# hku-mars/ImMesh

Measured on AMD Instinct MI355X. Metric: scans/sec (reg+mesh), 100k-pt scan into 10M-voxel map, higher is better.
Workload: dtype f64

## Files before the change

immesh_amd/csrc/c_api.cpp:

```cpp
#include "host_ctx.hpp"
#include "imu_host.hpp"
#include <cmath>
#include <new>

#define RP_ABORTED 1
static thread_local std::string g_create_error;
thread_local KProf* g_kprof = nullptr;



extern "C" {

void immesh_default_config(immesh_config* c) {
    std::memset(c, 0, sizeof(*c));
    c->voxel_size = 0.5; c->max_layer = 2;
    for (int i = 0; i < 5; i++) c->layer_init[i] = 5;
    c->max_points_size = 100; c->planer_threshold = 0.01; c->dept_err = 0.02; c->beam_err = 0.05; c->calib_laser = 0;
    c->sigma_num = 3.0; c->max_iter = 4;
    c->extR[0] = c->extR[4] = c->extR[8] = 1.0;
    c->extT[0] = 0.04165; c->extT[1] = 0.02326; c->extT[2] = -0.0284;
    c->mesh_min_spacing = 0.1; c->mesh_voxel = 0.4; c->mesh_region = 10.0; c->mesh_append_budget = 10000;
}

const char* immesh_create_error(void) { return g_create_error.c_str(); }
// ... 36 lines not shown

    const int64_t ns = g.cap_scan_points > 0 ? g.cap_scan_points : 600000;
    c->cap_scan = ns;
    A(c->d_pts_down, ns * 3); A(c->d_pts_raw, ns * 4);
    A(c->d_partials, ((ns + 63) / 64) * RES_NR); A(c->d_out48, RES_NV); A(c->d_done, 4);
    HIPCHK(c, hipMemsetAsync(c->d_done, 0, 16, c->stream));
    A(c->d_match, ns); A(c->d_mnode, ns); A(c->d_dis, ns); A(c->d_rinv, ns); A(c->d_normal, ns * 3);
    A(c->d_ptdata, ns * IM_PT_DOUBLES);
    A(c->d_key_a, ns); A(c->d_key_b, ns); A(c->d_idx_a, ns); A(c->d_idx_b, ns); A(c->d_idx_c, ns);
    A(c->d_slot, ns); A(c->d_slot_s, ns); A(c->d_seg_start, ns); A(c->d_nseg, 16); A(c->d_ds_out, ns * 3);
    c->sort_temp_bytes = std::max({sort_pairs_u64_temp_bytes((int)ns), sort_pairs_u32_temp_bytes((int)ns), exclusive_sum_temp_bytes((int)ns)}) + 256;
    { char* t; A(t, c->sort_temp_bytes); c->d_sort_temp = t; }
    A(c->p_key_a, ns); A(c->p_key_b, ns); A(c->p_idx_a, ns); A(c->p_idx_b, ns); A(c->p_idx_c, ns); A(c->p_seg, ns); A(c->p_nseg, 16); A(c->p_slot, ns); A(c->p_slot_s, ns); A(c->p_pool4, ns * 4);
    { char* t; A(t, c->sort_temp_bytes); c->p_sort_temp = t; }
    {
        unsigned long long cap = 1024; while (cap < 2ull * (unsigned long long)ns) cap <<= 1;
        char* t; A(t, cap * 16); c->p_htab = t; c->p_htab_cap = cap;
        launch_ds_table_reset(c->stream, t, cap);
        if ((rc = c->pinned(&c->h_ds_dyn, &c->d_ds_dyn, 1)) || (rc = c->pinned(&c->h_ds_info, &c->d_ds_info, 16))) return rc;
        HIPCHK(c, hipMemsetAsync(c->p_nseg, 0, 16 * sizeof(int32_t), c->stream));
    }
    {
        m.split_general = c->knobs.split_general >= 0 ? c->knobs.split_general : (g.max_layer >= 3 ? 1 : 0);
        A(m.sub_order, ns); A(m.sub_items, 2 * ns);
        HIPCHK(c, hipMemsetAsync(m.sub_items, 0, (size_t)2 * ns * sizeof(unsigned long long), c->stream));
    }
    A(c->d_dump_count, 2);
    A(c->d_touched, 2 * ns + 16);
    A(c->d_regstate, 1);
    A(c->d_epi, 8);
    HIPCHK(c, hipMemsetAsync(c->d_epi, 0, 32, c->stream));
    for (int q = 0; q < 2; q++) { A(c->d_rp_slots[q], RP_SLOT_DOUBLES); launch_fill_u64(c->stream, (unsigned long long*)c->d_rp_slots[q], RP_SLOT_SENTINEL, RP_SLOT_DOUBLES); }
    HIPCHK(c, hipMemsetAsync(c->d_regstate, 0, sizeof(RegState), c->stream));
    A(c->d_und_in, ns * 5); A(c->d_und_out, ns * 4); A(c->d_und_tab, 64 * 23 + 24);
#undef A
    if ((rc = c->pinned(&c->h_out48, &c->d_out48_host, RES_NV)) || (rc = c->pinned(&c->h_reg_out, &c->d_reg_out_host, REG_OUT_DOUBLES)) ||
        (rc = c->pinned(&c->h_epi_flag, &c->d_epi_flag_host, 8)) || (rc = c->pinned(&c->h_counters, &c->d_counters_host, 16))) return rc;
    return 0;
}


immesh_ctx* immesh_create(const immesh_config* cfg) {
    g_create_error.clear();
    if (!cfg) { g_create_error = "null config"; return nullptr; }
    int ndev = 0;
    hipError_t e = hipGetDeviceCount(&ndev);
// ... 678 lines not shown
```

immesh_amd/csrc/host_knobs.hpp:

```cpp
#pragma once
#include <hip/hip_runtime.h>
#include <algorithm>
#include <cstdlib>
#include <cstring>
#include <string>

struct Knobs {
    bool debug = false;
    bool debug_waits = false;
    std::string trace_file;
    int split_general = -1;
    bool no_priority = false;
    int mesh_cus = 0;
    int rp_blocks = 0;
    bool rp_force_abort = false;
    bool match_seq = false;
    bool host_ekf = false;
    bool serial_safe = false;
    bool serial_order = false;
    bool ds_radix = false;
    bool ds_no_gate = false;
    bool no_graph = false;
    int split_mode = 2;
    int mesh_room = 0;
    bool no_pipeline = false;
    int tri_stream = 1;
    int fused_wgs = 768;
    int list_div = 0;
    int mesh_grid_div = 1;

    static Knobs from_env(int mesh_npar) {
        auto on = [](const char* name) { return getenv(name) != nullptr; };
        auto num = [](const char* name, int unset) { const char* e = getenv(name); return e ? atoi(e) : unset; };
        Knobs k;
        k.debug = on("IMMESH_DEBUG"); k.debug_waits = on("IMMESH_DEBUG_WAITS");
        if (const char* e = getenv("IMMESH_TRACE_FILE")) k.trace_file = e;
        if (on("IMMESH_SPLIT_GENERAL")) k.split_general = num("IMMESH_SPLIT_GENERAL", 0);
        k.no_priority = on("IMMESH_NO_PRIORITY");
        k.mesh_cus = num("IMMESH_MESH_CUS", 0); if (k.mesh_cus < 8 || k.mesh_cus >= 1024) k.mesh_cus = 0;
        if (on("IMMESH_RP_BLOCKS")) k.rp_blocks = std::max(1, num("IMMESH_RP_BLOCKS", 0));
        k.rp_force_abort = on("IMMESH_RP_FORCE_ABORT"); k.match_seq = on("IMMESH_MATCH_SEQ"); k.host_ekf = on("IMMESH_HOST_EKF");
        k.serial_safe = on("IMMESH_SERIAL_SAFE"); k.serial_order = on("IMMESH_SERIAL_ORDER");
        k.ds_radix = on("IMMESH_DS_RADIX"); k.ds_no_gate = on("IMMESH_DS_NO_GATE");
        k.no_graph = on("IMMESH_NO_GRAPH");
        k.split_mode = on("IMMESH_NO_SPLIT") ? 0 : 2;
        if (on("IMMESH_SPLIT")) k.split_mode = num("IMMESH_SPLIT", 0) == 0 ? 0 : 1;
        if (on("IMMESH_MESH_ROOM")) k.mesh_room = std::min(std::max(num("IMMESH_MESH_ROOM", 0), 1), mesh_npar);
        k.no_pipeline = on("IMMESH_NO_PIPELINE");
        k.tri_stream = num("IMMESH_TRI_STREAM", 1);
        { const int v = num("IMMESH_FUSED_WGS", 0); k.fused_wgs = v >= 32 ? v : 768; }
        { const int v = num("IMMESH_LIST_DIV", 0); k.list_div = v >= 4 ? v : 0; }
        k.mesh_grid_div = std::max(1, num("IMMESH_MESH_GRID_DIV", 1));
        return k;
    }

    hipError_t make_stream(hipStream_t* s, int priority, bool maskable) const {
        if (!maskable || !mesh_cus) return hipStreamCreateWithPriority(s, hipStreamNonBlocking, priority);
        uint32_t mask[32];
        std::memset(mask, 0, sizeof(mask));
        for (int i = 0; i < mesh_cus; i++) mask[i >> 5] |= 1u << (i & 31);
        return hipExtStreamCreateWithCUMask(s, 32, mask);
    }
};
```

immesh_amd/csrc/reg_kernels.hip:

```cpp
#include <algorithm>
#include <cstdlib>
#include "regmap.hpp"
#include "kernels.hpp"
#include "prof.hpp"

using namespace imd;

struct PlaneRegs { double n[3], c[3], pv[21]; float d, radius; };
struct BestMatch { int node; int layer; double prob; bool ok; PlaneRegs P; };

IMD double plane_sigma(const double* pv, const double* J) {
    double tmp[6];
#pragma unroll
    for (int c = 0; c < 6; c++) {
        double s = 0;
#pragma unroll
        for (int r = 0; r < 6; r++) s += J[r] * pv[(r <= c) ? sym21_index(r, c) : sym21_index(c, r)];
        tmp[c] = s;
    }
    double sig = 0;
#pragma unroll
    for (int c = 0; c < 6; c++) sig += tmp[c] * J[c];
    return sig;
}
// ... 1184 lines not shown
#pragma unroll
        for (int k = 0; k < 3; k++) t[k] = q->t[k];
        transform_point(sp.extR, sp.extT, R, t, raw, world, i);
        return;
    }
    const int i = blockIdx.x * blockDim.x + threadIdx.x;
    if (i >= n) return;
    if (spd) {
#pragma unroll
        for (int k = 0; k < 9; k++) { sp.R[k] = spd->R[k]; sp.RextR[k] = spd->RextR[k]; sp.rot_var[k] = spd->rot_var[k]; sp.t_var[k] = spd->t_var[k]; }
#pragma unroll
        for (int k = 0; k < 3; k++) sp.t[k] = spd->t[k];
    }
    point_var_point(m, sp, pts, i, stride, mode, pt_data, sort_key, slot_out, pt_next);
}

__global__ void segment_heads_kernel(const uint32_t* __restrict__ sorted_slot, int n, int32_t* __restrict__ seg_start, int32_t* __restrict__ nseg) {
    const int i = blockIdx.x * blockDim.x + threadIdx.x;
    if (i >= n) return;
    if (sorted_slot[i] == 0xFFFFFFFFu) return;
    if (i == 0 || sorted_slot[i - 1] != sorted_slot[i]) seg_start[atomicAdd(nseg, 1)] = i;
}

struct WaveCtx { int lane; int64_t* stats; int root; bool shared = false; };

struct PlaneFit { double c[3], ev[3], U[9]; int imin, imax; bool planar; };
IMD double sel3(const int i, const double a, const double b, const double c) { return i == 0 ? a : (i == 1 ? b : c); }

template <class FE>
IMD void fit_eigen(FE&& for_each_point, const int n, const float planer_threshold, PlaneFit& f) {
    double s[9];
#pragma unroll
    for (int k = 0; k < 9; k++) s[k] = 0;
    for_each_point([&](const double* q) __attribute__((always_inline)) {
        const double x = q[0], y = q[1], z = q[2];
        s[0] += x; s[1] += y; s[2] += z;
        s[3] += x * x; s[4] += x * y; s[5] += x * z; s[6] += y * y; s[7] += y * z; s[8] += z * z;
    });
#pragma unroll
    for (int k = 0; k < 9; k++) s[k] = wave_sum_fast(s[k]);
    const double dn = (double)n;
    f.c[0] = s[0] / dn; f.c[1] = s[1] / dn; f.c[2] = s[2] / dn;
    double cov[9];
    cov[0] = s[3] / dn - f.c[0] * f.c[0]; cov[1] = s[4] / dn - f.c[0] * f.c[1]; cov[2] = s[5] / dn - f.c[0] * f.c[2];
    cov[3] = cov[1];                      cov[4] = s[6] / dn - f.c[1] * f.c[1]; cov[5] = s[7] / dn - f.c[1] * f.c[2];
    cov[6] = cov[2];                      cov[7] = cov[5];                      cov[8] = s[8] / dn - f.c[2] * f.c[2];
// ... 75 lines not shown
        const double Umin[3] = {sel3(imin, f.U[0], f.U[1], f.U[2]), sel3(imin, f.U[3], f.U[4], f.U[5]), sel3(imin, f.U[6], f.U[7], f.U[8])};
        if (lane < 21) {
            double v = 0;
#pragma unroll
            for (int k = 0; k < 21; k++) if (lane == k) v = pv[k];
            nr.p_var[lane] = v;
        }
        if (lane == 0) {
            const double evmin = sel3(imin, f.ev[0], f.ev[1], f.ev[2]);
            const double evmax = sel3(f.imax, f.ev[0], f.ev[1], f.ev[2]);
#pragma unroll
            for (int k = 0; k < 3; k++) { nr.p_center[k] = f.c[k]; nr.p_normal[k] = Umin[k]; }
            nr.min_eig = (float)evmin;
            nr.radius = (float)sqrt(evmax);
            nr.d = (float)(-(Umin[0] * f.c[0] + Umin[1] * f.c[1] + Umin[2] * f.c[2]));
        }
    } else if (lane == 0) {
#pragma unroll
        for (int k = 0; k < 3; k++) { nr.p_center[k] = f.c[k]; nr.p_normal[k] = 0.0; }
        nr.radius = 0.f;
    }
}

__device__ __noinline__ bool wave_init_plane(const RegMapDev& m, int nd, int n, const WaveCtx& w) {
    __builtin_amdgcn_fence(__ATOMIC_ACQUIRE, "workgroup");
    if (w.lane == 0 && w.stats) { atomicAdd((unsigned long long*)&w.stats[0], 1ull); atomicAdd((unsigned long long*)&w.stats[1], (unsigned long long)n); }
    PlaneFit f;
    double pv[21];
    const int lane = w.lane;
    if (n <= 128) {
        double P0[9], P1[9];
#pragma unroll
        for (int k = 0; k < 9; k++) { P0[k] = 0; P1[k] = 0; }
        if (lane < n) { const double* q = node_point_ptr(m, nd, lane);
#pragma unroll
            for (int k = 0; k < 9; k++) P0[k] = q[k]; }
        if (lane + 64 < n) { const double* q = node_point_ptr(m, nd, lane + 64);
#pragma unroll
            for (int k = 0; k < 9; k++) P1[k] = q[k]; }
        auto fe = [&](auto&& fn) __attribute__((always_inline)) { if (lane < n) fn(P0); if (lane + 64 < n) fn(P1); };
        fit_eigen(fe, n, m.planer_threshold, f);
        if (f.planar) fit_plane_var(fe, n, f, pv);
    } else {
        auto fe = [&](auto&& fn) __attribute__((always_inline)) {
            for (int i = lane; i < n; i += 64) {
                const double* q = node_point_ptr(m, nd, i);
                double P[9];
#pragma unroll
                for (int k = 0; k < 9; k++) P[k] = q[k];
                fn(P);
            }
        };
        fit_eigen(fe, n, m.planer_threshold, f);
        if (f.planar) fit_plane_var(fe, n, f, pv);
    }
    fit_store(m.nodes[nd], f, pv, lane);
    return f.planar;
}

__device__ bool wave_push_point(const RegMapDev& m, int nd, int n, const double* src, const WaveCtx& w) {
    int ok = 1;
    if (w.lane == 0 && (n % IM_CHUNK_PTS) == 0) ok = node_ensure_chunk(m, nd, n / IM_CHUNK_PTS) ? 1 : 0;
    ok = __shfl(ok, 0, 64);
    if (!ok) return false;
    __builtin_amdgcn_fence(__ATOMIC_RELEASE, "workgroup");
    __builtin_amdgcn_fence(__ATOMIC_ACQUIRE, "workgroup");
    if (w.lane < IM_PT_DOUBLES) {
        double* dst = node_point_ptr(m, nd, n);
        dst[w.lane] = src[w.lane];
    }
    __builtin_amdgcn_fence(__ATOMIC_RELEASE, "workgroup");
    return true;
}

IMD int octant_of(const double* q, const double* center) {
    return 4 * (q[0] > center[0] ? 1 : 0) + 2 * (q[1] > center[1] ? 1 : 0) + (q[2] > center[2] ? 1 : 0);
}
IMD int make_child(const RegMapDev& m, int nd, int oct) {
    const float ql = m.nodes[nd].quarter;
    const int xyz[3] = {(oct >> 2) & 1, (oct >> 1) & 1, oct & 1};
    double c[3];
#pragma unroll
    for (int k = 0; k < 3; k++) c[k] = m.nodes[nd].center[k] + (double)((float)(2 * xyz[k] - 1) * ql);
    const int layer = m.nodes[nd].layer + 1;
    const int child = node_alloc(m, layer, c, ql / 2, m.nodes[nd].key, m.nodes[nd].path | (oct << (3 * (layer - 1))));
    m.nodes[nd].child[oct] = child;
    return child;
}

__device__ void wave_init_octo_tree(const RegMapDev& m, int node, int* stack, const WaveCtx& w) {
    int sp = 0;
    if (w.lane == 0) stack[0] = node;
    sp = 1;
    while (sp > 0) {
        __builtin_amdgcn_fence(__ATOMIC_ACQUIRE, "workgroup");
        const int nd = __shfl(stack[sp - 1], 0, 64);
        sp--;
        const int n = m.nodes[nd].npts;
        const bool planar = wave_init_plane(m, nd, n, w);
        const int layer = m.nodes[nd].layer;
        if (w.lane == 0) {
            const int f0 = m.nodes[nd].flags;
            int f = f0 | NF_INIT;
            f = planar ? (f | NF_PLANE) : (f & ~NF_PLANE);
            node_set_flags(m, w.root, nd, f0, f, w.shared);
            m.nodes[nd].newpts = 0;
        }
        if (planar || layer >= m.max_layer) continue;
        const double ctr[3] = {m.nodes[nd].center[0], m.nodes[nd].center[1], m.nodes[nd].center[2]};
        int child_id[8], child_n[8];
#pragma unroll
        for (int k = 0; k < 8; k++) { child_id[k] = m.nodes[nd].child[k]; child_n[k] = child_id[k] >= 0 ? m.nodes[child_id[k]].npts : 0; }
        for (int base = 0; base < n; base += 64) {
// ... 24 lines not shown
#pragma unroll
                    for (int e = 0; e < IM_PT_DOUBLES; e++) dst[e] = q[e];
                }
                child_n[k] += cnt;
            }
        }
        __builtin_amdgcn_fence(__ATOMIC_RELEASE, "workgroup");
        if (w.lane == 0) {
#pragma unroll
            for (int k = 0; k < 8; k++)
                if (child_id[k] >= 0) { m.nodes[child_id[k]].npts = child_n[k]; m.nodes[child_id[k]].newpts = child_n[k]; }
            node_free_points(m, nd);
        }
#pragma unroll
        for (int k = 7; k >= 0; k--)
            if (child_id[k] >= 0 && child_n[k] > m.init_size[min(layer + 1, 4)]) {
                if (w.lane == 0) stack[sp] = child_id[k];
                sp++;
            }
        __builtin_amdgcn_fence(__ATOMIC_RELEASE, "workgroup");
    }
}

__device__ void wave_update_point(const RegMapDev& m, int root, const double* src, int* stack, const WaveCtx& w) {
    int nd = root;
    for (int depth = 0; depth < 8; depth++) {
        __builtin_amdgcn_fence(__ATOMIC_ACQUIRE, "workgroup");
        const int flags = m.nodes[nd].flags;
        const int layer = m.nodes[nd].layer;
        const int n = m.nodes[nd].npts;
        if (!(flags & NF_INIT)) {
            if (!wave_push_point(m, nd, n, src, w)) return;
            if (w.lane == 0) { m.nodes[nd].npts = n + 1; m.nodes[nd].newpts = m.nodes[nd].newpts + 1; }
            __builtin_amdgcn_fence(__ATOMIC_RELEASE, "workgroup");
            if (n + 1 > m.init_size[min(layer, 4)]) wave_init_octo_tree(m, nd, stack, w);
            return;
        }
        if (flags & NF_PLANE) {
            if (!(flags & NF_UPDATE_EN)) return;
            if (!wave_push_point(m, nd, n, src, w)) return;
            int newp = m.nodes[nd].newpts + 1;
            if (w.lane == 0) m.nodes[nd].npts = n + 1;
            __builtin_amdgcn_fence(__ATOMIC_RELEASE, "workgroup");
            if (newp > 5) {
                const bool planar = wave_init_plane(m, nd, n + 1, w);
                if (w.lane == 0) node_set_flags(m, w.root, nd, flags, planar ? (flags | NF_PLANE) : (flags & ~NF_PLANE), w.shared);
                newp = 0;
// ... 23 lines not shown
            if (child < 0) return;
            nd = child;
            continue;
        }
        if (!(flags & NF_UPDATE_EN)) return;
        if (!wave_push_point(m, nd, n, src, w)) return;
        int newp = m.nodes[nd].newpts + 1;
        if (w.lane == 0) m.nodes[nd].npts = n + 1;
        __builtin_amdgcn_fence(__ATOMIC_RELEASE, "workgroup");
        if (newp > 5) {
            const bool planar = wave_init_plane(m, nd, n + 1, w);
            if (w.lane == 0) node_set_flags(m, w.root, nd, flags, planar ? (flags | NF_PLANE) : (flags & ~NF_PLANE), w.shared);
            newp = 0;
        }
        if (w.lane == 0) {
            m.nodes[nd].newpts = newp;
            if (n + 1 > IM_G_MAX_POINTS) { m.nodes[nd].flags = m.nodes[nd].flags & ~NF_UPDATE_EN; node_free_points(m, nd); }
        }
        __builtin_amdgcn_fence(__ATOMIC_RELEASE, "workgroup");
        return;
    }
}

__device__ int wave_replay_planar_root(const RegMapDev& m, const int root, const int* order, const int cnt, const double* __restrict__ pt_data, const WaveCtx& w) {
    NodeRec& nd = m.nodes[root];
    int flags = nd.flags;
    const int layer = nd.layer;
    int npts = nd.npts, newp = nd.newpts;
    const int want = NF_INIT | NF_PLANE | NF_UPDATE_EN;
    if (layer == 0 && (flags & want) == (NF_INIT | NF_PLANE)) return cnt;
    if ((flags & want) != want || layer != 0 || npts + cnt > IM_INLINE_CHUNKS * IM_CHUNK_PTS) return 0;
    int chunks[IM_INLINE_CHUNKS];
#pragma unroll
    for (int k = 0; k < IM_INLINE_CHUNKS; k++) chunks[k] = nd.chunks[k];
    auto chunk_of = [&](int ci) { int c = chunks[0];
#pragma unroll
        for (int k = 1; k < IM_INLINE_CHUNKS; k++) { const int ck = chunks[k]; c = (ci == k) ? ck : c; }
        return c; };
    double s1[3] = {0, 0, 0}, s2[3] = {0, 0, 0};
    const bool will_refit = newp + cnt > 5;
    if (will_refit) {
        for (int i = w.lane; i < npts; i += 64) {
            const double* q = m.chunk_data + ((size_t)chunk_of(i / IM_CHUNK_PTS) * IM_CHUNK_PTS + (i % IM_CHUNK_PTS)) * IM_PT_DOUBLES;
#pragma unroll
            for (int a = 0; a < 3; a++) { const double v = q[a]; s1[a] += v; s2[a] += v * v; }
        }
#pragma unroll
// ... 57 lines not shown
                    }
                    j++;
                    break;
                }
            }
        }
        if (npts >= m.max_points_size) {
            if (last_refit_n) { write_header(); (void)wave_init_plane(m, root, last_refit_n, wq); last_refit_n = 0; }
            flags &= ~NF_UPDATE_EN;
            write_header();
            if (w.lane == 0) { node_free_points(m, root); nd.newpts = 0; }
            __builtin_amdgcn_fence(__ATOMIC_RELEASE, "workgroup");
            npts = 0; newp = 0;
            j++;
            break;
        }
    }
    if (header_dirty) write_header();
    if (last_refit_n) (void)wave_init_plane(m, root, last_refit_n, wq);
    if (w.lane == 0 && w.stats && n_ref) { atomicAdd((unsigned long long*)&w.stats[0], (unsigned long long)n_ref); atomicAdd((unsigned long long*)&w.stats[1], (unsigned long long)n_ref_pts); }
    return j;
}

__device__ int wave_replay_planar_node(const RegMapDev& m, const int node, const int* order, const int cnt, const double* __restrict__ pt_data, const WaveCtx& w) {
    NodeRec& nd = m.nodes[node];
    int flags = nd.flags;
    const int want = NF_INIT | NF_PLANE | NF_UPDATE_EN;
    if ((flags & want) == (NF_INIT | NF_PLANE)) return cnt;
    if ((flags & want) != want) return 0;
    int npts = nd.npts, newp = nd.newpts;
    double s1[3] = {0, 0, 0}, s2[3] = {0, 0, 0};
    const bool will_refit = newp + cnt > 5;
    if (will_refit) {
        for (int i = w.lane; i < npts; i += 64) {
            const double* q = node_point_ptr(m, node, i);
#pragma unroll
            for (int a = 0; a < 3; a++) { const double v = q[a]; s1[a] += v; s2[a] += v * v; }
        }
#pragma unroll
        for (int a = 0; a < 3; a++) { s1[a] = wave_sum(s1[a]); s2[a] = wave_sum(s2[a]); }
    }
    WaveCtx wq = w; wq.stats = nullptr;
    int last_refit_n = 0, n_ref = 0, j = 0;
    long long n_ref_pts = 0;
    auto write_counts = [&]() {
        if (w.lane == 0) { nd.npts = npts; nd.newpts = newp; }
        __builtin_amdgcn_fence(__ATOMIC_RELEASE, "workgroup");
// ... 67 lines not shown
    if (root < 0) return;
    w.root = root;
    if (mode == 0) {
        for (int j = start; j < n && sorted_slot[j] == slot; j++)
            wave_update_point(m, root, pt_data + (size_t)sorted_idx[j] * IM_PT_DOUBLES, stacks[wv], w);
    } else {
        int cnt = m.nodes[root].npts;
        for (int j = start; j < n && sorted_slot[j] == slot; j++) {
            if (!wave_push_point(m, root, cnt, pt_data + (size_t)sorted_idx[j] * IM_PT_DOUBLES, w)) return;
            cnt++;
        }
        if (w.lane == 0) { m.nodes[root].npts = cnt; m.nodes[root].newpts = cnt; }
        __builtin_amdgcn_fence(__ATOMIC_RELEASE, "workgroup");
        if (cnt > m.init_size[0]) wave_init_octo_tree(m, root, stacks[wv], w);
    }
}

#define RL_CAP 64
#define DBG_FUSED_OFF 64
#define DBG_FUSED_RECS 16384
#define DBG_RES_OFF (DBG_FUSED_OFF + DBG_FUSED_RECS * 8)
static_assert(DBG_RES_OFF + 8 * 512 * 8 == REG_DBG_WORDS, "the IMMESH_DEBUG buffer (kernels.hpp) holds the counters and both trace areas");
#define RF_PTS 128
__global__ __launch_bounds__(256, 3) void replay_fused_kernel(RegMapDev m, const int32_t* __restrict__ pt_next, const unsigned long long* __restrict__ sort_key,
                                                            const double* __restrict__ pt_data, int64_t* stats, uint32_t* __restrict__ general_list,
                                                            unsigned long long* __restrict__ dbg, unsigned long long* flag_dev, unsigned long long* flag_host,
                                                            unsigned long long flag_seq) {
    if (flag_dev && blockIdx.x == 0 && threadIdx.x == 0) {
        __hip_atomic_store(flag_dev, flag_seq, __ATOMIC_RELAXED, __HIP_MEMORY_SCOPE_AGENT);
        __hip_atomic_store(flag_host, flag_seq, __ATOMIC_RELAXED, __HIP_MEMORY_SCOPE_SYSTEM);
    }
    __shared__ unsigned long long skey[4][RL_CAP];
    __shared__ int sidx[4][RL_CAP];
    __shared__ int order[4][RL_CAP];
    __builtin_amdgcn_s_setprio(REG_UPD_PRIO);
    const int wv = threadIdx.x >> 6, lane = threadIdx.x & 63;
    const int t_first = blockIdx.x * 4 + wv, t_stride = gridDim.x * 4;
    uint32_t slot_first = m.touched[2 * (size_t)t_first];
    int root_first = (int)m.touched[2 * (size_t)t_first + 1];
    const int n_touched = m.counters[7];
#define FDBG(k) do { if (dbg) { const unsigned long long _t = __builtin_readcyclecounter(); if (tr) ((unsigned int*)tr)[4 + (k)] = (unsigned int)(_t - tprev); tprev = _t; } } while (0)
#define FEND(state, nref) do { if (tr) { tr[1] = __builtin_amdgcn_s_memrealtime(); tr[7] = (unsigned long long)((unsigned)cnt | ((unsigned)(nref) << 8) | ((unsigned)(state) << 16)); } } while (0)
    auto process = [&](const int t, const uint32_t slot, int root) __attribute__((always_inline)) {
    unsigned long long* const tr = (dbg && lane == 0 && t < DBG_FUSED_RECS) ? dbg + DBG_FUSED_OFF + (size_t)t * 8 : nullptr;
    unsigned long long tprev = dbg ? __builtin_readcyclecounter() : 0;
    if (tr) { tr[0] = __builtin_amdgcn_s_memrealtime(); tr[2] = tr[3] = tr[4] = tr[5] = tr[6] = tr[7] = 0; }
    if (root < 0) root = m.htab[slot].root;
    if (root < 0) return;
    FDBG(0);
    NodeRec& nd = m.nodes[root];
    const int flags = nd.flags, layer = nd.layer;
    const int npts = nd.npts, newp = nd.newpts;
    if (dbg) { asm volatile("s_waitcnt vmcnt(0)" ::: "memory"); FDBG(1); }
    int chunks[IM_INLINE_CHUNKS];
#pragma unroll
    for (int k = 0; k < IM_INLINE_CHUNKS; k++) chunks[k] = nd.chunks[k];
    if (dbg) { asm volatile("s_waitcnt vmcnt(0)" ::: "memory"); FDBG(2); }
    int cnt = 0;
    int ihead = (int)(unsigned int)(m.slot_head[slot] & 0xFFFFFFFFull);
    if (dbg) { asm volatile("s_waitcnt vmcnt(0)" ::: "memory"); FDBG(3); }
    for (int i = ihead; i >= 0; i = pt_next[i]) {
        if (cnt < RL_CAP && lane == 0) { skey[wv][cnt] = sort_key[i]; sidx[wv][cnt] = i; }
        cnt++;
    }
    FDBG(4);
    const int want = NF_INIT | NF_PLANE | NF_UPDATE_EN;
    if (layer == 0 && (flags & want) == (NF_INIT | NF_PLANE)) { FEND(1, 0); return; }
    const int ntot = npts + cnt;
    bool hand_over = cnt > RL_CAP || (flags & want) != want || layer != 0 || newp > 5 || ntot > RF_PTS || ntot >= m.max_points_size;
    if (!hand_over) {
        __builtin_amdgcn_fence(__ATOMIC_RELEASE, "workgroup");
        __builtin_amdgcn_wave_barrier();
        __builtin_amdgcn_fence(__ATOMIC_ACQUIRE, "workgroup");
        for (int e = lane; e < cnt; e += 64) {
            const unsigned long long k = skey[wv][e];
            const int id = sidx[wv][e];
            int rank = 0;
            for (int f = 0; f < cnt; f++) { const unsigned long long kf = skey[wv][f]; rank += (kf < k || (kf == k && sidx[wv][f] < id)) ? 1 : 0; }
            order[wv][rank] = id;
        }
        __builtin_amdgcn_fence(__ATOMIC_RELEASE, "workgroup");
        __builtin_amdgcn_wave_barrier();
        __builtin_amdgcn_fence(__ATOMIC_ACQUIRE, "workgroup");
        FDBG(5);
        auto chunk_of = [&](int ci) { int c = chunks[0];
#pragma unroll
            for (int k = 1; k < IM_INLINE_CHUNKS; k++) { const int ck = chunks[k]; c = (ci == k) ? ck : c; }
            return c; };
        const int n_ref = (newp + cnt) / 6;
        double P0[9], P1[9];
#pragma unroll
        for (int k = 0; k < 9; k++) { P0[k] = 0; P1[k] = 0; }
        {
// ... 54 lines not shown
                    for (int k = 0; k < 9; k++) d[k] = P0[k]; }
                if (q1 >= npts && q1 < ntot) { double* d = m.chunk_data + ((size_t)chunk_of(q1 >> 4) * IM_CHUNK_PTS + (q1 & 15)) * IM_PT_DOUBLES;
#pragma unroll
                    for (int k = 0; k < 9; k++) d[k] = P1[k]; }
            }
            if (lane == 0) {
                nd.npts = ntot; nd.newpts = (newp + cnt) % 6;
#pragma unroll
                for (int k = 0; k < IM_INLINE_CHUNKS; k++) nd.chunks[k] = chunks[k];
                if (n_ref) { int64_t* sh = stats + 16 + (size_t)(t & 63) * 16; atomicAdd((unsigned long long*)&sh[0], (unsigned long long)n_ref); atomicAdd((unsigned long long*)&sh[1], (unsigned long long)n_ref_pts); }
            }
            FDBG(8);
            if (n_ref > 0) {
                double pv[21];
                auto fe = [&](auto&& fn) __attribute__((always_inline)) { if (lane < n_last) fn(P0); if (lane + 64 < n_last) fn(P1); };
                fit_plane_var(fe, n_last, fit, pv);
                fit_store(nd, fit, pv, lane);
            }
            FDBG(9);
            FEND(2, n_ref);
            return;
        }
    }
    if (lane == 0) general_list[atomicAdd(&m.counters[10], 1)] = slot;
    FEND(3, 0);
    };
    for (int t = t_first; t < n_touched; t += t_stride) {
        if (t != t_first) { slot_first = m.touched[2 * (size_t)t]; root_first = (int)m.touched[2 * (size_t)t + 1]; }
        process(t, slot_first, root_first);
    }
#undef FDBG
#undef FEND
}

__device__ bool replay_split_root(const RegMapDev& m, const int root, const int* order, const int cnt, const double* __restrict__ pt_data, const WaveCtx& w);
__device__ bool replay_split_leaves(const RegMapDev& m, const int root, const int* order, const int cnt, const double* __restrict__ pt_data, const WaveCtx& w, int* s_key, int* s_first);
__global__ __launch_bounds__(256) void replay_list_kernel(RegMapDev m, const int32_t* __restrict__ pt_next, const unsigned long long* __restrict__ sort_key,
                                                           const double* __restrict__ pt_data, int64_t* stats, int32_t* __restrict__ big_idx, int32_t* __restrict__ big_order,
                                                           unsigned long long* __restrict__ dbg, const uint32_t* __restrict__ work, const int32_t* __restrict__ n_work) {
    __shared__ unsigned long long skey[4][RL_CAP];
    __shared__ int sidx[4][RL_CAP];
    __shared__ int order[4][RL_CAP];
    __shared__ int stacks[4][48];
    __builtin_amdgcn_s_setprio(REG_UPD_PRIO);
    const int wv = threadIdx.x >> 6;
    const int nw = *n_work;
    WaveCtx w; w.lane = threadIdx.x & 63; w.stats = stats;
    for (int t = blockIdx.x * 4 + wv; t < nw; t += gridDim.x * 4) {
        const uint32_t slot = work[t];
        const int root = m.htab[slot].root;
        if (root < 0) continue;
        w.root = root;
        const unsigned long long tdbg0 = dbg ? __builtin_readcyclecounter() : 0;
        __builtin_amdgcn_wave_barrier();
        int cnt = 0;
        for (int i = (int)(unsigned int)(m.slot_head[slot] & 0xFFFFFFFFull); i >= 0; i = pt_next[i]) {
            if (cnt < RL_CAP && w.lane == 0) { skey[wv][cnt] = sort_key[i]; sidx[wv][cnt] = i; }
            cnt++;
        }
        if (cnt > RL_CAP) {
            int base = 0;
            if (w.lane == 0) base = atomicAdd(&m.counters[9], cnt);
            base = __shfl(base, 0, 64);
            if (w.lane == 0) { int k = 0; for (int i = (int)(unsigned int)(m.slot_head[slot] & 0xFFFFFFFFull); i >= 0; i = pt_next[i]) big_idx[base + k++] = i; }
            __builtin_amdgcn_fence(__ATOMIC_RELEASE, "agent");
            __builtin_amdgcn_wave_barrier();
            __builtin_amdgcn_fence(__ATOMIC_ACQUIRE, "agent");
            for (int e = w.lane; e < cnt; e += 64) {
                const int id = big_idx[base + e];
                const unsigned long long k = sort_key[id];
                int rank = 0;
                for (int f = 0; f < cnt; f++) { const int idf = big_idx[base + f]; const unsigned long long kf = sort_key[idf]; rank += (kf < k || (kf == k && idf < id)) ? 1 : 0; }
                big_order[base + rank] = id;
            }
            __builtin_amdgcn_fence(__ATOMIC_RELEASE, "agent");
            __builtin_amdgcn_wave_barrier();
            __builtin_amdgcn_fence(__ATOMIC_ACQUIRE, "agent");
            if (replay_split_root(m, root, big_order + base, cnt, pt_data, w)) continue;
            int jb = wave_replay_planar_root(m, root, big_order + base, cnt, pt_data, w);
            if (jb == 0) jb = wave_replay_planar_node(m, root, big_order + base, cnt, pt_data, w);
            for (int j = jb; j < cnt; j++) wave_update_point(m, root, pt_data + (size_t)big_order[base + j] * IM_PT_DOUBLES, stacks[wv], w);
            continue;
        }
        __builtin_amdgcn_fence(__ATOMIC_RELEASE, "workgroup");
        __builtin_amdgcn_wave_barrier();
        __builtin_amdgcn_fence(__ATOMIC_ACQUIRE, "workgroup");
        for (int e = w.lane; e < cnt; e += 64) {
            const unsigned long long k = skey[wv][e];
            const int id = sidx[wv][e];
            int rank = 0;
            for (int f = 0; f < cnt; f++) { const unsigned long long kf = skey[wv][f]; rank += (kf < k || (kf == k && sidx[wv][f] < id)) ? 1 : 0; }
            order[wv][rank] = id;
        }
        __builtin_amdgcn_fence(__ATOMIC_RELEASE, "workgroup");
        __builtin_amdgcn_wave_barrier();
        __builtin_amdgcn_fence(__ATOMIC_ACQUIRE, "workgroup");
        if (replay_split_leaves(m, root, order[wv], cnt, pt_data, w, (int*)skey[wv], sidx[wv])) continue;
        if (replay_split_root(m, root, order[wv], cnt, pt_data, w)) continue;
        const unsigned long long tdbg1 = dbg ? __builtin_readcyclecounter() : 0;
        int jf = wave_replay_planar_root(m, root, order[wv], cnt, pt_data, w);
        if (jf == 0) jf = wave_replay_planar_node(m, root, order[wv], cnt, pt_data, w);
        for (int j = jf; j < cnt; j++) wave_update_point(m, root, pt_data + (size_t)order[wv][j] * IM_PT_DOUBLES, stacks[wv], w);
        if (dbg && w.lane == 0) {
            const unsigned long long t2 = __builtin_readcyclecounter();
            atomicMax(&dbg[jf == cnt ? 8 : 9], ((t2 - tdbg0) << 16) | (unsigned long long)cnt);
            atomicAdd(&dbg[jf == cnt ? 10 : 11], t2 - tdbg1);
            atomicAdd(&dbg[jf == cnt ? 12 : 13], 1ull);
            atomicAdd(&dbg[14], tdbg1 - tdbg0);
        }
    }
}

#define SPLIT_MISSING 0x40000000
__device__ __noinline__ bool replay_split_leaves(const RegMapDev& m, const int root, const int* order, const int cnt, const double* __restrict__ pt_data, const WaveCtx& w, int* s_key, int* s_first) {
    const NodeRec& nr = m.nodes[root];
    const int flags = nr.flags;
    if (!m.split_general || cnt < 2 || cnt > RL_CAP || !(flags & NF_INIT) || (flags & NF_PLANE) || nr.layer >= m.max_layer || m.cap_nodes >= (1 << 26)) return false;
    if (w.lane == 0 && nr.npts != 0) node_free_points(m, root);
    const int lane = w.lane;
    int key = -1;
    if (lane < cnt) {
        const double* q = pt_data + (size_t)order[lane] * IM_PT_DOUBLES;
        const double qx = q[0], qy = q[1], qz = q[2];
        int nd = root;
        for (int depth = 0; depth < 8; depth++) {
            const NodeRec& r = m.nodes[nd];
            const int f = r.flags, layer = r.layer, npts = r.npts;
            if (!((f & NF_INIT) && !(f & NF_PLANE) && layer < m.max_layer && (npts == 0 || nd == root))) { key = nd; break; }
            const int oct = 4 * (qx > r.center[0] ? 1 : 0) + 2 * (qy > r.center[1] ? 1 : 0) + (qz > r.center[2] ? 1 : 0);
            const int child = r.child[oct];
            if (child < 0) { key = nd | (oct << 26) | SPLIT_MISSING; break; }
            nd = child;
// ... 182 lines not shown
    if (!(a.pad & 4) && m.cap_nodes < (1 << 26)) KLAUNCH(residual_persistent_kernel<true>, dim3(nb + 1), dim3(256), 0, s, m, a, rs, pts, n, slots, slots_next, a.max_iter * RP_MAX_BLOCKS * RES_NR, host_counters, reg_out, ticket, o_match, o_node,
            o_dis, o_rinv, o_normal, ep);
    else KLAUNCH(residual_persistent_kernel<false>, dim3(nb + 1), dim3(256), 0, s, m, a, rs, pts, n, slots, slots_next, a.max_iter * RP_MAX_BLOCKS * RES_NR, host_counters, reg_out, ticket, o_match, o_node,
            o_dis, o_rinv, o_normal, ep);
}
int residual_persistent_resident_blocks(int device) {
    int per_cu = 0, cus = 0;
    if (hipOccupancyMaxActiveBlocksPerMultiprocessor(&per_cu, residual_persistent_kernel<true>, 256, 0) != hipSuccess) { (void)hipGetLastError(); per_cu = 1; }
    if (hipDeviceGetAttribute(&cus, hipDeviceAttributeMultiprocessorCount, device) != hipSuccess) { (void)hipGetLastError(); cus = 0; }
    return std::max(1, per_cu) * cus;
}
void launch_ekf_step(hipStream_t s, const RegIterArgs& a, RegState* rs, const double* sums48, double* reg_out, double ticket) {
    KLAUNCH(ekf_step_kernel, dim3(1), dim3(64), 0, s, a, rs, sums48, reg_out, ticket);
}
void launch_point_var(hipStream_t s, const RegMapDev& m, const ScanParams& sp, const ScanParams* spd, const float* pts, int n, int stride, int mode, double* pt_data,
                      unsigned long long* sort_key, uint32_t* slot, int32_t* pt_next, const float* raw_xyzi, float* world_xyzi, int n_raw) {
    const int nb_pv = (n + 255) / 256, nb_x = raw_xyzi ? (n_raw + 255) / 256 : 0;
    KLAUNCH(point_var_kernel, dim3(nb_pv + nb_x), dim3(256), 0, s, m, sp, spd, pts, n, stride, mode, pt_data, sort_key, slot, pt_next, (const float4*)raw_xyzi,
            (float4*)world_xyzi, n_raw, nb_pv);
}
void launch_replay_lists(hipStream_t s, const RegMapDev& m, const int32_t* pt_next, const unsigned long long* sort_key, const double* pt_data, int n,
                         int64_t* stats, int32_t* host_counters, int32_t* big_idx, int32_t* big_order, uint32_t* general_list, unsigned long long* dbg, bool with_tail,
                         unsigned long long* flag_dev, unsigned long long* flag_host, unsigned long long flag_seq, int fused_wgs, int list_div_knob) {
    KLAUNCH(replay_fused_kernel, dim3(std::min((n + 3) / 4, fused_wgs)), dim3(256), 0, s, m, pt_next, sort_key, pt_data, stats, general_list, dbg, flag_dev, flag_host, flag_seq);
    const int list_div = list_div_knob ? list_div_knob : (m.split_general ? 32 : 128);
    const int nb_list = std::min(std::max((n + list_div - 1) / list_div, 32), 4096);
    KLAUNCH(replay_list_kernel, dim3(nb_list), dim3(256), 0, s, m, pt_next, sort_key, pt_data, stats, big_idx, big_order, dbg, (const uint32_t*)general_list,
            (const int32_t*)(m.counters + 10));
    if (m.split_general) KLAUNCH(replay_sub_kernel, dim3(std::min(std::max((n + 15) / 16, 32), 2048)), dim3(256), 0, s, m, pt_data, stats);
    if (with_tail) KLAUNCH(merge_free_tail_kernel, dim3(1), dim3(256), 0, s, m, host_counters);
}
void launch_map_update_tail(hipStream_t s, const RegMapDev& m, int32_t* host_counters) { KLAUNCH(merge_free_tail_kernel, dim3(1), dim3(256), 0, s, m, host_counters); }
void launch_segment_heads(hipStream_t s, const uint32_t* sorted_slot, int n, int32_t* seg_start, int32_t* nseg) {
    (void)hipMemsetAsync(nseg, 0, sizeof(int32_t), s);
    KLAUNCH(segment_heads_kernel, dim3((n + 255) / 256), dim3(256), 0, s, sorted_slot, n, seg_start, nseg);
}
void launch_replay(hipStream_t s, const RegMapDev& m, const uint32_t* sorted_slot, const int32_t* sorted_idx, const double* pt_data, int n,
                   const int32_t* seg_start, const int32_t* nseg, int max_segments, int mode, int64_t* stats) {
    KLAUNCH(replay_kernel, dim3((max_segments + 3) / 4), dim3(256), 0, s, m, sorted_slot, sorted_idx, pt_data, n, seg_start, nseg, mode, stats);
    KLAUNCH(merge_free_kernel, dim3(64), dim3(256), 0, s, m);
    KLAUNCH(merge_free_finish_kernel, dim3(1), dim3(1), 0, s, m);
}
void launch_dump_planes(hipStream_t s, const RegMapDev& m, PlaneRecDev* out, long long cap, unsigned long long* count) {
    (void)hipMemsetAsync(count, 0, sizeof(unsigned long long), s);
    KLAUNCH(dump_planes_kernel, dim3(1024), dim3(256), 0, s, m, out, cap, count);
}
void launch_fill_u64(hipStream_t s, unsigned long long* p, unsigned long long v, size_t n) {
    KLAUNCH(fill_u64_kernel, dim3(2048), dim3(256), 0, s, p, v, n);
}
void launch_iota(hipStream_t s, int32_t* p, int n) { KLAUNCH(iota_kernel, dim3((n + 255) / 256), dim3(256), 0, s, p, n); }
```

immesh_amd/csrc/regmap.hpp:

```cpp
#pragma once
#include "dev_math.hpp"

#define IM_CHUNK_PTS 16
#define IM_PT_DOUBLES 9
#define IM_INLINE_CHUNKS 8
#define IM_EXT_CHUNKS 2048
#define IM_LEAF_SLOTS 15
#define IM_G_MAX_POINTS 1000

#define NF_INIT 1
#define NF_PLANE 2
#define NF_UPDATE_EN 4

struct alignas(64) NodeRec {
    int32_t child[8];
    int32_t flags, layer, npts, newpts;
    float quarter, d, radius, min_eig;
    double center[3];
    double p_center[3];
    double p_normal[3];
    double p_var[21];
    int32_t chunks[IM_INLINE_CHUNKS];
    int32_t ext, path;
    unsigned long long key;
    int32_t leaf_head;
    int32_t lock;
    unsigned long long pad[3];
};
static_assert(sizeof(NodeRec) == 384, "NodeRec layout");

struct HashEnt { unsigned long long key; int32_t root; int32_t pad; };

struct RegMapDev {
    HashEnt* htab;
    uint64_t hmask;
    NodeRec* nodes;
    double* chunk_data;
    int32_t* ext_tables;
    int32_t* counters;
    int32_t* free_ready;
    int32_t* free_pending;
    int32_t* leaf_chunks;
    int32_t cap_leaf_chunks;
    unsigned long long* slot_head;
    uint32_t* touched;
    int32_t split_general;
    int32_t* sub_order;
    unsigned long long* sub_items;
    int32_t upd_seq;
    int32_t shard_rank, shard_world, shard_brick_log2, shard_scheme;
    int32_t cap_nodes, cap_chunks, cap_ext;
    int32_t max_layer, max_points_size, init_size[5];
    float planer_threshold;
    float voxel_size_f;
    double voxel_size_d;
};

namespace imd {

IMD int sym21_index(int r, int c) {
    return r * 6 - (r * (r - 1)) / 2 + (c - r);
}

IMHD int brick_owner(int scheme, int world, int64_t bx, int64_t by, int64_t bz, uint64_t packed) {
    if (scheme == 1 || world % 3 == 0 || world % 5 == 0) return (int)(hash64(packed) % (uint64_t)world);
    const int64_t c = (bx + 3 * by + 5 * bz) % (int64_t)world;
    return (int)(c < 0 ? c + world : c);
}
IMD int shard_owner(const RegMapDev& m, int64_t kx, int64_t ky, int64_t kz) {
// ... 158 lines not shown
```

Baseline: 6034.

## Finish handed-over voxels inside the fused replay kernel instead of a list launch

When split_general is off (the default for max_layer<3), voxels the fast path cannot handle are no longer appended to a global list for a second replay_list_kernel launch. Each wave now records its own leftovers and processes them at the end of replay_fused_kernel with a shared, inlined wave_replay_voxel routine. The several wave helpers are also force-inlined. This removes a kernel launch and the atomic list, but puts the slow-path work and its register and LDS use into the fused kernel, which may lower occupancy or leave load imbalance across waves.

```diff
diff --git a/immesh_amd/csrc/c_api.cpp b/immesh_amd/csrc/c_api.cpp
--- a/immesh_amd/csrc/c_api.cpp
+++ b/immesh_amd/csrc/c_api.cpp
@@ -82,6 +82,7 @@
     }
     {
         m.split_general = c->knobs.split_general >= 0 ? c->knobs.split_general : (g.max_layer >= 3 ? 1 : 0);
+        m.list_launch = c->knobs.list_launch ? 1 : 0;
         A(m.sub_order, ns); A(m.sub_items, 2 * ns);
         HIPCHK(c, hipMemsetAsync(m.sub_items, 0, (size_t)2 * ns * sizeof(unsigned long long), c->stream));
     }
diff --git a/immesh_amd/csrc/host_knobs.hpp b/immesh_amd/csrc/host_knobs.hpp
--- a/immesh_amd/csrc/host_knobs.hpp
+++ b/immesh_amd/csrc/host_knobs.hpp
@@ -26,6 +26,7 @@
     bool no_pipeline = false;
     int tri_stream = 1;
     int fused_wgs = 768;
+    bool list_launch = false;
     int list_div = 0;
     int mesh_grid_div = 1;
 
@@ -48,7 +49,8 @@
         if (on("IMMESH_MESH_ROOM")) k.mesh_room = std::min(std::max(num("IMMESH_MESH_ROOM", 0), 1), mesh_npar);
         k.no_pipeline = on("IMMESH_NO_PIPELINE");
         k.tri_stream = num("IMMESH_TRI_STREAM", 1);
-        { const int v = num("IMMESH_FUSED_WGS", 0); k.fused_wgs = v >= 32 ? v : 768; }
+        { const int v = num("IMMESH_FUSED_WGS", 0); k.fused_wgs = v >= 1 ? v : 768; }
+        k.list_launch = num("IMMESH_LIST_LAUNCH", 0) != 0;
         { const int v = num("IMMESH_LIST_DIV", 0); k.list_div = v >= 4 ? v : 0; }
         k.mesh_grid_div = std::max(1, num("IMMESH_MESH_GRID_DIV", 1));
         return k;
diff --git a/immesh_amd/csrc/reg_kernels.hip b/immesh_amd/csrc/reg_kernels.hip
--- a/immesh_amd/csrc/reg_kernels.hip
+++ b/immesh_amd/csrc/reg_kernels.hip
@@ -1230,6 +1230,7 @@
     if (i == 0 || sorted_slot[i - 1] != sorted_slot[i]) seg_start[atomicAdd(nseg, 1)] = i;
 }
 
+#define WAVE_FN __device__ __attribute__((always_inline)) inline
 struct WaveCtx { int lane; int64_t* stats; int root; bool shared = false; };
 
 struct PlaneFit { double c[3], ev[3], U[9]; int imin, imax; bool planar; };
@@ -1351,7 +1352,7 @@
     }
 }
 
-__device__ __noinline__ bool wave_init_plane(const RegMapDev& m, int nd, int n, const WaveCtx& w) {
+WAVE_FN bool wave_init_plane(const RegMapDev& m, int nd, int n, const WaveCtx& w) {
     __builtin_amdgcn_fence(__ATOMIC_ACQUIRE, "workgroup");
     if (w.lane == 0 && w.stats) { atomicAdd((unsigned long long*)&w.stats[0], 1ull); atomicAdd((unsigned long long*)&w.stats[1], (unsigned long long)n); }
     PlaneFit f;
@@ -1387,7 +1388,7 @@
     return f.planar;
 }
 
-__device__ bool wave_push_point(const RegMapDev& m, int nd, int n, const double* src, const WaveCtx& w) {
+WAVE_FN bool wave_push_point(const RegMapDev& m, int nd, int n, const double* src, const WaveCtx& w) {
     int ok = 1;
     if (w.lane == 0 && (n % IM_CHUNK_PTS) == 0) ok = node_ensure_chunk(m, nd, n / IM_CHUNK_PTS) ? 1 : 0;
     ok = __shfl(ok, 0, 64);
@@ -1417,7 +1418,7 @@
     return child;
 }
 
-__device__ void wave_init_octo_tree(const RegMapDev& m, int node, int* stack, const WaveCtx& w) {
+WAVE_FN void wave_init_octo_tree(const RegMapDev& m, int node, int* stack, const WaveCtx& w) {
     int sp = 0;
     if (w.lane == 0) stack[0] = node;
     sp = 1;
@@ -1488,7 +1489,7 @@
     }
 }
 
-__device__ void wave_update_point(const RegMapDev& m, int root, const double* src, int* stack, const WaveCtx& w) {
+WAVE_FN void wave_update_point(const RegMapDev& m, int root, const double* src, int* stack, const WaveCtx& w) {
     int nd = root;
     for (int depth = 0; depth < 8; depth++) {
         __builtin_amdgcn_fence(__ATOMIC_ACQUIRE, "workgroup");
@@ -1558,7 +1559,7 @@
     }
 }
 
-__device__ int wave_replay_planar_root(const RegMapDev& m, const int root, const int* order, const int cnt, const double* __restrict__ pt_data, const WaveCtx& w) {
+WAVE_FN int wave_replay_planar_root(const RegMapDev& m, const int root, const int* order, const int cnt, const double* __restrict__ pt_data, const WaveCtx& w) {
     NodeRec& nd = m.nodes[root];
     int flags = nd.flags;
     const int layer = nd.layer;
@@ -1662,7 +1663,7 @@
     return j;
 }
 
-__device__ int wave_replay_planar_node(const RegMapDev& m, const int node, const int* order, const int cnt, const double* __restrict__ pt_data, const WaveCtx& w) {
+WAVE_FN int wave_replay_planar_node(const RegMapDev& m, const int node, const int* order, const int cnt, const double* __restrict__ pt_data, const WaveCtx& w) {
     NodeRec& nd = m.nodes[node];
     int flags = nd.flags;
     const int want = NF_INIT | NF_PLANE | NF_UPDATE_EN;
@@ -1776,8 +1777,71 @@
 #define DBG_RES_OFF (DBG_FUSED_OFF + DBG_FUSED_RECS * 8)
 static_assert(DBG_RES_OFF + 8 * 512 * 8 == REG_DBG_WORDS, "the IMMESH_DEBUG buffer (kernels.hpp) holds the counters and both trace areas");
 #define RF_PTS 128
+__device__ bool replay_split_root(const RegMapDev& m, const int root, const int* order, const int cnt, const double* __restrict__ pt_data, const WaveCtx& w);
+__device__ bool replay_split_leaves(const RegMapDev& m, const int root, const int* order, const int cnt, const double* __restrict__ pt_data, const WaveCtx& w, int* s_key, int* s_first);
+template <bool SPLIT>
+WAVE_FN void wave_replay_voxel(const RegMapDev& m, const uint32_t slot, const int root, unsigned long long* skey, int* sidx,
+                               int* order, int* stack, const int32_t* __restrict__ pt_next, const unsigned long long* __restrict__ sort_key, const double* __restrict__ pt_data,
+                               int32_t* __restrict__ big_idx, int32_t* __restrict__ big_order, unsigned long long* __restrict__ dbg, const unsigned long long t0, const WaveCtx& w) {
+    __builtin_amdgcn_wave_barrier();
+    int cnt = 0;
+    for (int i = (int)(unsigned int)(m.slot_head[slot] & 0xFFFFFFFFull); i >= 0; i = pt_next[i]) {
+        if (cnt < RL_CAP && w.lane == 0) { skey[cnt] = sort_key[i]; sidx[cnt] = i; }
+        cnt++;
+    }
+    const int* ord = order;
+    if (cnt > RL_CAP) {
+        int base = 0;
+        if (w.lane == 0) base = atomicAdd(&m.counters[9], cnt);
+        base = __shfl(base, 0, 64);
+        if (w.lane == 0) { int k = 0; for (int i = (int)(unsigned int)(m.slot_head[slot] & 0xFFFFFFFFull); i >= 0; i = pt_next[i]) big_idx[base + k++] = i; }
+        __builtin_amdgcn_fence(__ATOMIC_RELEASE, "agent");
+        __builtin_amdgcn_wave_barrier();
+        __builtin_amdgcn_fence(__ATOMIC_ACQUIRE, "agent");
+        for (int e = w.lane; e < cnt; e += 64) {
+            const int id = big_idx[base + e];
+            const unsigned long long k = sort_key[id];
+            int rank = 0;
+            for (int f = 0; f < cnt; f++) { const int idf = big_idx[base + f]; const unsigned long long kf = sort_key[idf]; rank += (kf < k || (kf == k && idf < id)) ? 1 : 0; }
+            big_order[base + rank] = id;
+        }
+        __builtin_amdgcn_fence(__ATOMIC_RELEASE, "agent");
+        __builtin_amdgcn_wave_barrier();
+        __builtin_amdgcn_fence(__ATOMIC_ACQUIRE, "agent");
+        ord = big_order + base;
+    } else {
+        __builtin_amdgcn_fence(__ATOMIC_RELEASE, "workgroup");
+        __builtin_amdgcn_wave_barrier();
+        __builtin_amdgcn_fence(__ATOMIC_ACQUIRE, "workgroup");
+        for (int e = w.lane; e < cnt; e += 64) {
+            const unsigned long long k = skey[e];
+            const int id = sidx[e];
+            int rank = 0;
+            for (int f = 0; f < cnt; f++) { const unsigned long long kf = skey[f]; rank += (kf < k || (kf == k && sidx[f] < id)) ? 1 : 0; }
+            order[rank] = id;
+        }
+        __builtin_amdgcn_fence(__ATOMIC_RELEASE, "workgroup");
+        __builtin_amdgcn_wave_barrier();
+        __builtin_amdgcn_fence(__ATOMIC_ACQUIRE, "workgroup");
+    }
+    if (SPLIT && replay_split_leaves(m, root, ord, cnt, pt_data, w, (int*)skey, sidx)) return;
+    if (SPLIT && replay_split_root(m, root, ord, cnt, pt_data, w)) return;
+    const unsigned long long t1 = dbg ? __builtin_readcyclecounter() : 0;
+    int jf = wave_replay_planar_root(m, root, ord, cnt, pt_data, w);
+    if (jf == 0) jf = wave_replay_planar_node(m, root, ord, cnt, pt_data, w);
+    for (int j = jf; j < cnt; j++) wave_update_point(m, root, pt_data + (size_t)ord[j] * IM_PT_DOUBLES, stack, w);
+    if (dbg && w.lane == 0 && cnt <= RL_CAP) {
+        const unsigned long long t2 = __builtin_readcyclecounter();
+        atomicMax(&dbg[jf == cnt ? 8 : 9], ((t2 - t0) << 16) | (unsigned long long)cnt);
+        atomicAdd(&dbg[jf == cnt ? 10 : 11], t2 - t1);
+        atomicAdd(&dbg[jf == cnt ? 12 : 13], 1ull);
+        atomicAdd(&dbg[14], t1 - t0);
+    }
+}
+
 __global__ __launch_bounds__(256, 3) void replay_fused_kernel(RegMapDev m, const int32_t* __restrict__ pt_next, const unsigned long long* __restrict__ sort_key,
                                                             const double* __restrict__ pt_data, int64_t* stats, uint32_t* __restrict__ general_list,
+                                                            int32_t* __restrict__ big_idx, int32_t* __restrict__ big_order,
                                                             unsigned long long* __restrict__ dbg, unsigned long long* flag_dev, unsigned long long* flag_host,
                                                             unsigned long long flag_seq) {
     if (flag_dev && blockIdx.x == 0 && threadIdx.x == 0) {
@@ -1787,14 +1851,17 @@
     __shared__ unsigned long long skey[4][RL_CAP];
     __shared__ int sidx[4][RL_CAP];
     __shared__ int order[4][RL_CAP];
+    __shared__ int stacks[4][48];
     __builtin_amdgcn_s_setprio(REG_UPD_PRIO);
     const int wv = threadIdx.x >> 6, lane = threadIdx.x & 63;
+    const bool finish_here = !m.split_general && !m.list_launch;
     const int t_first = blockIdx.x * 4 + wv, t_stride = gridDim.x * 4;
     uint32_t slot_first = m.touched[2 * (size_t)t_first];
     int root_first = (int)m.touched[2 * (size_t)t_first + 1];
     const int n_touched = m.counters[7];
 #define FDBG(k) do { if (dbg) { const unsigned long long _t = __builtin_readcyclecounter(); if (tr) ((unsigned int*)tr)[4 + (k)] = (unsigned int)(_t - tprev); tprev = _t; } } while (0)
 #define FEND(state, nref) do { if (tr) { tr[1] = __builtin_amdgcn_s_memrealtime(); tr[7] = (unsigned long long)((unsigned)cnt | ((unsigned)(nref) << 8) | ((unsigned)(state) << 16)); } } while (0)
+    int n_mine = 0;
     auto process = [&](const int t, const uint32_t slot, int root) __attribute__((always_inline)) {
     unsigned long long* const tr = (dbg && lane == 0 && t < DBG_FUSED_RECS) ? dbg + DBG_FUSED_OFF + (size_t)t * 8 : nullptr;
     unsigned long long tprev = dbg ? __builtin_readcyclecounter() : 0;
@@ -1822,7 +1889,7 @@
     if (layer == 0 && (flags & want) == (NF_INIT | NF_PLANE)) { FEND(1, 0); return; }
     const int ntot = npts + cnt;
     bool hand_over = cnt > RL_CAP || (flags & want) != want || layer != 0 || newp > 5 || ntot > RF_PTS || ntot >= m.max_points_size;
-    if (!hand_over) {
+    if (__builtin_expect(!hand_over, 1)) {
         __builtin_amdgcn_fence(__ATOMIC_RELEASE, "workgroup");
         __builtin_amdgcn_wave_barrier();
         __builtin_amdgcn_fence(__ATOMIC_ACQUIRE, "workgroup");
@@ -1923,19 +1990,34 @@
             return;
         }
     }
-    if (lane == 0) general_list[atomicAdd(&m.counters[10], 1)] = slot;
+    if (!finish_here) { if (lane == 0) general_list[atomicAdd(&m.counters[10], 1)] = slot; }
+    else { if (lane == 0) general_list[t_first + n_mine * t_stride] = (uint32_t)t; n_mine++; }
     FEND(3, 0);
     };
     for (int t = t_first; t < n_touched; t += t_stride) {
         if (t != t_first) { slot_first = m.touched[2 * (size_t)t]; root_first = (int)m.touched[2 * (size_t)t + 1]; }
         process(t, slot_first, root_first);
     }
+    if (__builtin_expect(n_mine > 0, 0)) {
+        WaveCtx w; w.lane = lane; w.stats = stats;
+        for (int j = 0; j < n_mine; j++) {
+            int t = 0;
+            if (lane == 0) t = (int)general_list[t_first + j * t_stride];
+            t = __shfl(t, 0, 64);
+            const uint32_t slot = m.touched[2 * (size_t)t];
+            int root = (int)m.touched[2 * (size_t)t + 1];
+            if (root < 0) root = m.htab[slot].root;
+            if (root < 0) continue;
+            w.root = root;
+            const unsigned long long t0 = dbg ? __builtin_readcyclecounter() : 0;
+            wave_replay_voxel<false>(m, slot, root, skey[wv], sidx[wv], order[wv], stacks[wv], pt_next, sort_key, pt_data, big_idx, big_order, dbg, t0, w);
+            if (dbg && lane == 0 && t < DBG_FUSED_RECS) dbg[DBG_FUSED_OFF + (size_t)t * 8 + 1] = __builtin_amdgcn_s_memrealtime();
+        }
+    }
 #undef FDBG
 #undef FEND
 }
 
-__device__ bool replay_split_root(const RegMapDev& m, const int root, const int* order, const int cnt, const double* __restrict__ pt_data, const WaveCtx& w);
-__device__ bool replay_split_leaves(const RegMapDev& m, const int root, const int* order, const int cnt, const double* __restrict__ pt_data, const WaveCtx& w, int* s_key, int* s_first);
 __global__ __launch_bounds__(256) void replay_list_kernel(RegMapDev m, const int32_t* __restrict__ pt_next, const unsigned long long* __restrict__ sort_key,
                                                            const double* __restrict__ pt_data, int64_t* stats, int32_t* __restrict__ big_idx, int32_t* __restrict__ big_order,
                                                            unsigned long long* __restrict__ dbg, const uint32_t* __restrict__ work, const int32_t* __restrict__ n_work) {
@@ -1953,62 +2035,7 @@
         if (root < 0) continue;
         w.root = root;
         const unsigned long long tdbg0 = dbg ? __builtin_readcyclecounter() : 0;
-        __builtin_amdgcn_wave_barrier();
-        int cnt = 0;
-        for (int i = (int)(unsigned int)(m.slot_head[slot] & 0xFFFFFFFFull); i >= 0; i = pt_next[i]) {
-            if (cnt < RL_CAP && w.lane == 0) { skey[wv][cnt] = sort_key[i]; sidx[wv][cnt] = i; }
-            cnt++;
-        }
-        if (cnt > RL_CAP) {
-            int base = 0;
-            if (w.lane == 0) base = atomicAdd(&m.counters[9], cnt);
-            base = __shfl(base, 0, 64);
-            if (w.lane == 0) { int k = 0; for (int i = (int)(unsigned int)(m.slot_head[slot] & 0xFFFFFFFFull); i >= 0; i = pt_next[i]) big_idx[base + k++] = i; }
-            __builtin_amdgcn_fence(__ATOMIC_RELEASE, "agent");
-            __builtin_amdgcn_wave_barrier();
-            __builtin_amdgcn_fence(__ATOMIC_ACQUIRE, "agent");
-            for (int e = w.lane; e < cnt; e += 64) {
-                const int id = big_idx[base + e];
-                const unsigned long long k = sort_key[id];
-                int rank = 0;
-                for (int f = 0; f < cnt; f++) { const int idf = big_idx[base + f]; const unsigned long long kf = sort_key[idf]; rank += (kf < k || (kf == k && idf < id)) ? 1 : 0; }
-                big_order[base + rank] = id;
-            }
-            __builtin_amdgcn_fence(__ATOMIC_RELEASE, "agent");
-            __builtin_amdgcn_wave_barrier();
-            __builtin_amdgcn_fence(__ATOMIC_ACQUIRE, "agent");
-            if (replay_split_root(m, root, big_order + base, cnt, pt_data, w)) continue;
-            int jb = wave_replay_planar_root(m, root, big_order + base, cnt, pt_data, w);
-            if (jb == 0) jb = wave_replay_planar_node(m, root, big_order + base, cnt, pt_data, w);
-            for (int j = jb; j < cnt; j++) wave_update_point(m, root, pt_data + (size_t)big_order[base + j] * IM_PT_DOUBLES, stacks[wv], w);
-            continue;
-        }
-        __builtin_amdgcn_fence(__ATOMIC_RELEASE, "workgroup");
-        __builtin_amdgcn_wave_barrier();
-        __builtin_amdgcn_fence(__ATOMIC_ACQUIRE, "workgroup");
-        for (int e = w.lane; e < cnt; e += 64) {
-            const unsigned long long k = skey[wv][e];
-            const int id = sidx[wv][e];
-            int rank = 0;
-            for (int f = 0; f < cnt; f++) { const unsigned long long kf = skey[wv][f]; rank += (kf < k || (kf == k && sidx[wv][f] < id)) ? 1 : 0; }
-            order[wv][rank] = id;
-        }
-        __builtin_amdgcn_fence(__ATOMIC_RELEASE, "workgroup");
-        __builtin_amdgcn_wave_barrier();
-        __builtin_amdgcn_fence(__ATOMIC_ACQUIRE, "workgroup");
-        if (replay_split_leaves(m, root, order[wv], cnt, pt_data, w, (int*)skey[wv], sidx[wv])) continue;
-        if (replay_split_root(m, root, order[wv], cnt, pt_data, w)) continue;
-        const unsigned long long tdbg1 = dbg ? __builtin_readcyclecounter() : 0;
-        int jf = wave_replay_planar_root(m, root, order[wv], cnt, pt_data, w);
-        if (jf == 0) jf = wave_replay_planar_node(m, root, order[wv], cnt, pt_data, w);
-        for (int j = jf; j < cnt; j++) wave_update_point(m, root, pt_data + (size_t)order[wv][j] * IM_PT_DOUBLES, stacks[wv], w);
-        if (dbg && w.lane == 0) {
-            const unsigned long long t2 = __builtin_readcyclecounter();
-            atomicMax(&dbg[jf == cnt ? 8 : 9], ((t2 - tdbg0) << 16) | (unsigned long long)cnt);
-            atomicAdd(&dbg[jf == cnt ? 10 : 11], t2 - tdbg1);
-            atomicAdd(&dbg[jf == cnt ? 12 : 13], 1ull);
-            atomicAdd(&dbg[14], tdbg1 - tdbg0);
-        }
+        wave_replay_voxel<true>(m, slot, root, skey[wv], sidx[wv], order[wv], stacks[wv], pt_next, sort_key, pt_data, big_idx, big_order, dbg, tdbg0, w);
     }
 }
 
@@ -2237,11 +2264,14 @@
 void launch_replay_lists(hipStream_t s, const RegMapDev& m, const int32_t* pt_next, const unsigned long long* sort_key, const double* pt_data, int n,
                          int64_t* stats, int32_t* host_counters, int32_t* big_idx, int32_t* big_order, uint32_t* general_list, unsigned long long* dbg, bool with_tail,
                          unsigned long long* flag_dev, unsigned long long* flag_host, unsigned long long flag_seq, int fused_wgs, int list_div_knob) {
-    KLAUNCH(replay_fused_kernel, dim3(std::min((n + 3) / 4, fused_wgs)), dim3(256), 0, s, m, pt_next, sort_key, pt_data, stats, general_list, dbg, flag_dev, flag_host, flag_seq);
+    KLAUNCH(replay_fused_kernel, dim3(std::min((n + 3) / 4, fused_wgs)), dim3(256), 0, s, m, pt_next, sort_key, pt_data, stats, general_list, big_idx, big_order, dbg, flag_dev, flag_host,
+            flag_seq);
+    if (m.split_general || m.list_launch) {
     const int list_div = list_div_knob ? list_div_knob : (m.split_general ? 32 : 128);
     const int nb_list = std::min(std::max((n + list_div - 1) / list_div, 32), 4096);
     KLAUNCH(replay_list_kernel, dim3(nb_list), dim3(256), 0, s, m, pt_next, sort_key, pt_data, stats, big_idx, big_order, dbg, (const uint32_t*)general_list,
             (const int32_t*)(m.counters + 10));
+    }
     if (m.split_general) KLAUNCH(replay_sub_kernel, dim3(std::min(std::max((n + 15) / 16, 32), 2048)), dim3(256), 0, s, m, pt_data, stats);
     if (with_tail) KLAUNCH(merge_free_tail_kernel, dim3(1), dim3(256), 0, s, m, host_counters);
 }
diff --git a/immesh_amd/csrc/regmap.hpp b/immesh_amd/csrc/regmap.hpp
--- a/immesh_amd/csrc/regmap.hpp
+++ b/immesh_amd/csrc/regmap.hpp
@@ -45,6 +45,7 @@
     unsigned long long* slot_head;
     uint32_t* touched;
     int32_t split_general;
+    int32_t list_launch;
     int32_t* sub_order;
     unsigned long long* sub_items;
     int32_t upd_seq;
```

New measurement: 5915. 2.0% lower.
